# Mattdl/CLsurvey

Hardware: AMD Instinct MI355X
Metric: images/sec (train+importance pass), EWC small_VGG9 Tiny-ImageNet task batch (higher is better)
Workload: dtype f32 (bf16x6 split operands on the conv fwd/bwd-data matrix products, fp32 accumulate); 1 GPU; EWC small_VGG9_cl_128_128, Tiny-ImageNet shapes (3x64x64, 20 classes), batch 200: train step + Fisher step (BASELINE configs[1]); batch=200, parallelism=1 GPU

## Files before the change

### clsurvey_amd/_lib.py

```python
import ctypes as C
import os

_HERE = os.path.dirname(os.path.abspath(__file__))
LIB_PATH = os.path.join(_HERE, "libclhip.so")

_p = C.c_void_p
_i = C.c_int
_f = C.c_float
_z = C.c_size_t
_l = C.c_long


class HatParam(C.Structure):
    _fields_ = [("theta", _p), ("grad", _p), ("buf", _p), ("mask_back", _p), ("n", _z), ("is_emb", _i), ("reserved", _i)]


class HatGateJob(C.Structure):
    _fields_ = [("emb_row", _p), ("gate", _p), ("mask_pre", _p), ("n", _i), ("reserved", _i)]


class HatLayer(C.Structure):
    _fields_ = [("w", _p), ("gate_in", _p), ("out", _p), ("K", _z), ("C", _z), ("R", _z)]


# ... 99 lines not shown
    "clhip_hat_emb_grads_multi": (_i, [_p, _i, _f, _f, _f, _p, _p]),
    "clhip_pathnet_ws": (_z, [_p, _i]),
    "clhip_pathnet_pack_multi": (_i, [_p, _i, _p, _z, _p, _z, _p]),
    "clhip_pathnet_fold_grads_multi": (_i, [_p, _i, _p, _z, _p, _z, _p, _z, _p]),
    "clhip_pathnet_sgd_step": (_i, [_p, _i, _p, _p, _p, _z, _f, _f, _f, _f, _i, _p, _z, _p]),
    "clhip_softmax_ce_slice": (_i, [_p, _p, _i, _i, _i, _i, _i, _p, _p, _p, _p]),
    "clhip_net_loss_step_slice": (_i, [_p, _p, _p, _p, _p, _i, _i, _i, _i, _p, _p, _p, _p, _p]),
    "clhip_axpy": (_i, [_p, _p, _z, _f, _i, _p]),
    "clhip_gem_gram_ws": (_z, [_i]),
    "clhip_gem_gram": (_i, [_p, _z, C.POINTER(_i), _i, _z, _p, _p, _z, _p]),
    "clhip_gem_project": (_i, [_p, _z, C.POINTER(_i), C.POINTER(_f), _i, _p, _p, _z, _p]),
    "clhip_gem_qp": (_i, [_p, _i, C.c_double, C.c_double, _p, _p, _p]),
    "clhip_gem_project_dev": (_i, [_p, _z, C.POINTER(_i), _p, _p, _i, _p, _p, _z, _p]),
    "clhip_net_create": (_i, [C.POINTER(LayerDesc), _i, _i, _i, _i, _i, C.POINTER(_p)]),
    "clhip_net_set_dropout": (_i, [_p, _i, _p, _l]),
    "clhip_net_set_bn": (_i, [_p, _i, _p, _p, _f, _f]),
    "clhip_net_set_training": (_i, [_p, _i]),
    "clhip_net_probe": (_i, [_p, _i]),
    "clhip_net_probe_read": (_i, [_p, C.POINTER(_f), C.POINTER(_i)]),
    "clhip_net_layer_input": (_i, [_p, _i, _p, _p]),
    "clhip_net_layer_pool_idx": (_i, [_p, _i, _p, _p]),
    "clhip_net_prepared_weights": (_i, [_p, _p, _p]),
    "clhip_net_edge_grid_count": (_i, [_p]),
    "clhip_net_layer_paths": (_i, [_p, _i]),
    "clhip_net_probe_kind": (_i, [_p, _i, _i]),
    "clhip_net_set_input_grad": (_i, [_p, _i, _p]),
    "clhip_sigmoid_fwd": (_i, [_p, _p, _z, _p]),
    "clhip_sigmoid_bwd": (_i, [_p, _p, _p, _z, _p]),
    "clhip_mse_mean": (_i, [_p, _p, _z, _f, _p, _p, _p]),
    "clhip_adadelta_step": (_i, [_p, _p, _p, _p, _z, _f, _f, _f, _f, _p]),
    "clhip_bn_ws": (_z, [_i]),
    "clhip_bn_fwd": (_i, [_p, _p, _p, _p, _p, _p, _p, _p, _i, _i, _i, _i, _f, _f, _i, _p, _z, _p]),
    "clhip_bn_bwd": (_i, [_p, _p, _p, _p, _p, _p, _p, _p, _p, _i, _i, _i, _i, _i, _p, _z, _p]),
    "clhip_net_destroy": (None, [_p]),
    "clhip_net_workspace_bytes": (_z, [_p]),
    "clhip_net_num_classes": (_i, [_p]),
    "clhip_net_forward": (_i, [_p, _p, _p, _i, _p, _p, _p]),
    "clhip_net_backward": (_i, [_p, _p, _p, _p, _i, _p, _p, _p]),
    "clhip_net_loss_step": (_i, [_p, _p, _p, _p, _p, _i, _i, _p, _p, _p, _p, _p]),
    "clhip_rehearsal_assemble": (_i, [_p, _p, _i, _z, _p, _p, _l, _l, _i, _p, _i, _p, _p, _p]),
    "clhip_rehearsal_assemble_crop_flip": (_i, [_p, _p, _i, _i, _i, _i, _i, _i, _p, _l, _p, _p, _p, _l, _l, _i, _p, _p, _i, _p, _p, _p]),
    "clhip_rehearsal_assemble_resized_crop_flip": (_i, [_p, _p, _i, _i, _i, _i, _i, _i, _p, _l, _p, _p, _p, _l, _l, _i, _p, _p, _i, _p, _p, _p]),
    "clhip_loss_segments": (_i, [_p, _p, _p, _i, _i, _i, _p, _i, _f, _p, _p, _p, _p]),
    "clhip_net_loss_step_loss_segments": (_i, [_p, _p, _p, _p, _p, _p, _i, _i, _p, _i, _f, _p, _p, _p, _p, _p]),
    "clhip_gather_tasks": (_i, [_p, _i, _z, _p, _i, _p, _p, _p]),
    "clhip_slice_argmax_count": (_i, [_p, _i, _i, _p, _i, _p, _p, _p, _p, _p]),
# ... 52 lines not shown
```

### clsurvey_amd/csrc/common.hpp

```cpp
#pragma once
#include <hip/hip_runtime.h>
#include <stdint.h>
#include <stddef.h>
#include "../../include/clhip.h"

#define CLHIP_LAUNCH_CHECK()                          \
    do {                                              \
        hipError_t e__ = hipGetLastError();           \
        if (e__ != hipSuccess) return (int)e__;       \
    } while (0)

static inline hipStream_t as_stream(void* s) { return reinterpret_cast<hipStream_t>(s); }

static inline bool aligned16(const void* p) { return (reinterpret_cast<uintptr_t>(p) & 15u) == 0; }

static inline int ew_grid(size_t work_items, int block) {
    size_t g = (work_items + block - 1) / block;
    if (g < 1) g = 1;
    if (g > 2048) g = 2048;
    return (int)g;
}

static __device__ __attribute__((aligned(16))) float clhip_zero16[4] = {0.f, 0.f, 0.f, 0.f};

// ... 100 lines not shown
int clhip_internal_fc_fwd_partial(const float* x, const float* w, int M, int I, int O, void* ws, size_t ws_bytes, int* live,
                                  hipStream_t s);

#define CLHIP_WGRAD_JOBS_MAX 32
struct clhip_wgrad_job { const float* part; float* dw; float* db; int K, C, splits; int taps; };
int clhip_internal_conv3x3_wgrad_partial(const float* x, const float* dy, const uint8_t* unpool_idx, float* dw, float* db, int N,
                                         int C, int K, int H, int W, void* ws, size_t ws_bytes, void* stream, clhip_wgrad_job* job);
int clhip_internal_wgrad_reduce_multi(const clhip_wgrad_job* jobs, int n, hipStream_t s);

bool clhip_internal_convkk_ok(int N, int Cin, int Cout, int H, int W, int R, int S, int stride, int pad);
int clhip_internal_convkk(int mode, const float* in, const float* w, const float* bias, const float* mask_src, float* out, int N,
                          int Cin, int Cout, int H, int W, int relu, hipStream_t s);

struct clhip_wino_wt { const float* w; float* U; int Ko, Ci, mode, pad; };
int clhip_internal_wino_weights(const clhip_wino_wt* jobs, int n, hipStream_t s);
int clhip_internal_weight_images(const clhip_wino_wt* wino_jobs, int n_wino, const clhip_wino_wt* bs_jobs, int n_bs, hipStream_t s);
int clhip_internal_c3w64_pool_weight_images(const float* x, const float* w, const float* b, float* y_pool, uint8_t* idx_u8, int N, int C,
                                            int K, int H, int W, const clhip_wino_wt* wino_jobs, int n_wino, const clhip_wino_wt* bs_jobs,
                                            int n_bs, int wt_first, hipStream_t s);
int clhip_internal_wino_conv_u(int mode, const float* in, const float* U, const float* bias, const float* mask_src, float* out,
                               uint8_t* pool_idx, int unpool, int N, int Cin, int Cout, int H, int W, int relu, hipStream_t s);
bool clhip_internal_wino_ok(int Cin, int Cout, int H, int W);
size_t clhip_internal_wino_ws(int Cin, int Cout);
bool clhip_internal_bs_ok(int Cin, int Cout, int H, int W);
bool clhip_internal_bs_preferred(int Cin, int Cout, int H, int W);
bool clhip_internal_bs5_preferred(int Cin, int Cout, int H, int W);
size_t clhip_internal_bs5_ws(int Cin, int Cout);
int clhip_internal_bs5_conv_u(int mode, const float* in, const void* wimg, const float* bias, const float* mask_src, float* out, int N,
                              int Cin, int Cout, int H, int W, int relu, hipStream_t s);
size_t clhip_internal_bs_ws(int Cin, int Cout);
int clhip_internal_bs_weights(const clhip_wino_wt* jobs, int n, hipStream_t s);
int clhip_internal_bs_conv_u(int mode, const float* in, const void* wimg, const float* bias, const float* mask_src, float* out,
                             uint8_t* pool_idx, int unpool, int N, int Cin, int Cout, int H, int W, int relu, hipStream_t s);
bool clhip_internal_bs5_wgrad_ok(int N, int C, int K, int H, int W);
size_t clhip_internal_bs5_wgrad_ws(int N, int C, int K, int H, int W);
int clhip_internal_bs5_wgrad(const float* x, const float* dy, float* dw, float* db, int N, int C, int K, int H, int W, void* ws,
                             size_t ws_bytes, hipStream_t s);
size_t clhip_internal_bs3k_wgrad_ws(int N, int C, int K, int H, int W);
int clhip_internal_bs3k_wgrad(const float* x, const float* dy, float* dw, float* db, int N, int C, int K, int H, int W, void* ws,
                              size_t ws_bytes, hipStream_t s);
bool clhip_internal_bs_wgrad_ok(int C, int K, int H, int W);
bool clhip_internal_bs_wgrad_preferred(int C, int K, int H, int W, int pooled);
size_t clhip_internal_bs_wgrad_ws(int N, int C, int K, int H, int W);
int clhip_internal_bs_wgrad_partial(const float* x, const float* dy, const uint8_t* unpool_idx, float* dw, float* db, int N, int C, int K,
                                    int H, int W, void* ws, size_t ws_bytes, hipStream_t s, clhip_wgrad_job* job);
bool clhip_internal_wino_wgrad_ok(int C, int K, int H, int W);
// ... 11 lines not shown
```

### clsurvey_amd/csrc/engine.hip

```cpp
#include <vector>
#include <cstdlib>
#include <new>
#include "common.hpp"

namespace {

struct LayerPlan {
    int type;
    int cin, cout, relu, pool;
    long w_off, b_off;
    int h, w;
    int ks, st, pd;
    int oh, ow;
    int pk, ps;
    int ph, pw;
    size_t in_elems, out_elems, pool_elems;
    size_t act_off;
    size_t pool_off;
    size_t idx_off;
    int bn;
    long bn_w_off, bn_b_off;
    size_t z_off;
    size_t stat_off;
    float* rmean; float* rvar; float bn_momentum, bn_eps;
// ... 10 lines not shown
    const float* extra_grad;
    const float* drop;
    long drop_stride;
    int has_drop_buf;
    size_t drop_off;
};

constexpr long long WINO_MIN_UNITS = 640;
constexpr long long WINO16_MIN_UNITS = 384;
static bool wino_small_wgrad() { return true; }

static bool wino_enabled() {
    const char* e = std::getenv("CLHIP_WINO");
    return !(e && e[0] == '0');
}

constexpr unsigned PROBE_RING = 64;
#ifndef CLHIP_EDGE_GRIDS_DEFAULT
#define CLHIP_EDGE_GRIDS_DEFAULT 1
#endif
#ifndef CLHIP_OVERLAP_DEFAULT
#define CLHIP_OVERLAP_DEFAULT 0
#endif

struct NetPlan {
    std::vector<LayerPlan> layers;
    int max_batch, in_c, in_h, in_w, n_classes;
    size_t in_elems;
    size_t acts_floats;
    size_t idx_bytes;
    size_t grad_floats;
    size_t scratch_bytes;
    size_t wino_bytes;
    size_t off_wino;
    size_t off_s2d;
    int s2d_fresh_n;
    size_t total_bytes;
    size_t off_acts, off_idx, off_g0, off_g1, off_scratch, off_dlogits, off_loss, off_fcdz, off_wg;
    int training;
    int n_wg;
    int fc_first;
    bool fc_fused;
    clhip_fc_chain chain;
    int probe_layer;
    int probe_kind;
    unsigned probe_count;
    std::vector<hipEvent_t> probe_ev;
    bool fc_tail, no_combo;
    unsigned* tail_counter;
    size_t off_rows;
    int edge_grids;
    unsigned edge_count;
    bool overlap;
    int overlap_mode;
    hipStream_t side;
    std::vector<hipEvent_t> ev_dy, ev_wg;
    ~NetPlan() {
        for (hipEvent_t e : ev_dy) (void)hipEventDestroy(e);
        for (hipEvent_t e : ev_wg) (void)hipEventDestroy(e);
        if (side) (void)hipStreamDestroy(side);
        if (tail_counter) (void)hipFree(tail_counter);
        for (hipEvent_t e : probe_ev) (void)hipEventDestroy(e);
    }
};

inline size_t align_up(size_t v, size_t a) { return (v + a - 1) / a * a; }

__global__ void drop_scale_kernel(float* __restrict__ h, const float* __restrict__ mask, long stride, int feat, size_t total) {
    for (size_t i = blockIdx.x * (size_t)blockDim.x + threadIdx.x; i < total; i += (size_t)gridDim.x * blockDim.x) {
        const size_t n = i / feat, f = i - n * feat;
        h[i] *= mask[n * stride + f];
    }
}

__global__ void add_inplace_kernel(float* __restrict__ a, const float* __restrict__ b, size_t n) {
// ... 209 lines not shown
    p->total_bytes = off;
    p->training = 1;
    p->overlap = false;
    p->side = nullptr;
    const char* ov = getenv("CLHIP_WGRAD_OVERLAP");
    bool any_bn = false;
    for (const LayerPlan& L : p->layers) any_bn = any_bn || L.bn;
    p->overlap_mode = (ov && ov[0] == '1') ? 1 : (ov && ov[0] == '2') ? 2 : CLHIP_OVERLAP_DEFAULT;
    if (p->overlap_mode && !any_bn) {
        if (hipStreamCreateWithFlags(&p->side, hipStreamNonBlocking) == hipSuccess) {
            p->overlap = true;
            p->ev_dy.resize(n_layers); p->ev_wg.resize(n_layers);
            for (int i = 0; i < n_layers && p->overlap; ++i)
                if (hipEventCreateWithFlags(&p->ev_dy[i], hipEventDisableTiming) != hipSuccess ||
                    hipEventCreateWithFlags(&p->ev_wg[i], hipEventDisableTiming) != hipSuccess) p->overlap = false;
        } else {
            (void)hipGetLastError();
            p->side = nullptr;
        }
    }
    p->edge_count = 0;
    const char* eg = getenv("CLHIP_EDGE_GRIDS");
    p->edge_grids = (eg && eg[0] >= '0' && eg[0] <= '2' && !eg[1]) ? eg[0] - '0' : CLHIP_EDGE_GRIDS_DEFAULT;
    p->probe_layer = -1;
    p->probe_kind = 0;
    p->probe_count = 0;
    p->fc_tail = false;
    p->no_combo = false;
    p->tail_counter = nullptr;
    const char* tl = getenv("CLHIP_FC_TAIL");
    if (tl && tl[0] == '0') p->no_combo = true;
    if (p->fc_fused && !(tl && tl[0] == '0') && clhip_internal_fc_tail_ok(&p->chain) &&
        max_batch <= 1024) {
        if (hipMalloc(reinterpret_cast<void**>(&p->tail_counter), 256) == hipSuccess &&
            hipMemset(p->tail_counter, 0, 256) == hipSuccess) {
            p->fc_tail = true;
        } else {
            (void)hipGetLastError();
            if (p->tail_counter) { (void)hipFree(p->tail_counter); p->tail_counter = nullptr; }
        }
    }
    *out_handle = p;
    return 0;
}

int clhip_net_set_dropout(void* handle, int layer, const float* mask, long row_stride) {
// ... 16 lines not shown
    NetPlan* p = static_cast<NetPlan*>(handle);
    if (!p || layer <= 0 || layer >= (int)p->layers.size() || !ws_float_off || !in_elems) return CLHIP_EINVAL;
    const LayerPlan& P = p->layers[layer - 1];
    *ws_float_off = p->off_acts / sizeof(float) + ((P.type == 0 && P.pool) ? P.pool_off : P.act_off);
    *in_elems = p->layers[layer].in_elems;
    return 0;
}

int clhip_net_layer_pool_idx(void* handle, int layer, size_t* ws_byte_off, size_t* elems) {
    NetPlan* p = static_cast<NetPlan*>(handle);
    if (!p || layer < 0 || layer >= (int)p->layers.size() || !ws_byte_off || !elems) return CLHIP_EINVAL;
    const LayerPlan& L = p->layers[layer];
    if (L.type != 0 || !L.pool) return CLHIP_EINVAL;
    *ws_byte_off = p->off_idx + L.idx_off;
    *elems = L.pool_elems;
    return 0;
}

int clhip_net_edge_grid_count(void* handle) {
    NetPlan* p = static_cast<NetPlan*>(handle);
    return p ? (int)(p->edge_count & 0x7fffffffu) : CLHIP_EINVAL;
}

int clhip_net_prepared_weights(void* handle, size_t* ws_byte_off, size_t* bytes) {
    NetPlan* p = static_cast<NetPlan*>(handle);
    if (!p || !ws_byte_off || !bytes) return CLHIP_EINVAL;
    *ws_byte_off = p->off_wino;
    *bytes = p->wino_bytes;
    return 0;
}

int clhip_net_layer_paths(void* handle, int layer) {
    NetPlan* p = static_cast<NetPlan*>(handle);
    if (!p || layer < 0 || layer >= (int)p->layers.size()) return CLHIP_EINVAL;
    const LayerPlan& L = p->layers[layer];
    const bool defer_capable = p->n_wg > 0 && !(p->overlap && p->overlap_mode == 1);
    if (L.type == 1) {
        bool tail = p->fc_tail && layer > p->fc_first;
        for (size_t i = p->fc_first + 1; tail && i < p->layers.size(); ++i)
            if (p->layers[i].drop || p->layers[i].extra_grad) tail = false;
        return (tail ? 64 : 0) | ((p->fc_fused && layer >= p->fc_first) ? 128 : 0);
    }
    return (L.wino_f ? 1 : 0) | (L.wino_d ? 2 : 0) | ((L.wino_w && defer_capable) ? 4 : 0) | ((L.bs_f || L.bs5_f) ? 8 : 0) |
           ((L.bs_d || L.bs5_d) ? 16 : 0) | ((L.bs_w && defer_capable) ? 32 : 0);
}

// ... 81 lines not shown
}

static void wino_collect(const NetPlan* p, const float* params, char* base, bool fwd, bool bwd, std::vector<clhip_wino_wt>& jobs,
                         std::vector<clhip_wino_wt>& bsjobs) {
    jobs.reserve(2 * p->layers.size());
    bsjobs.reserve(2 * p->layers.size());
    for (const LayerPlan& L : p->layers) {
        if (L.type != 0) continue;
        if (fwd && L.wino_f)
            (L.bs_f ? bsjobs : jobs).push_back(clhip_wino_wt{params + L.w_off, reinterpret_cast<float*>(base + p->off_wino + L.wino_uf), L.cout, L.cin, 0, 0});
        if (bwd && L.wino_d)
            (L.bs_d ? bsjobs : jobs).push_back(clhip_wino_wt{params + L.w_off, reinterpret_cast<float*>(base + p->off_wino + L.wino_ud), L.cin, L.cout, 1, 0});
        if (fwd && L.bs5_f)
            bsjobs.push_back(clhip_wino_wt{params + L.w_off, reinterpret_cast<float*>(base + p->off_wino + L.wino_uf), L.cout, L.cin, 0, 5});
        if (bwd && L.bs5_d)
            bsjobs.push_back(clhip_wino_wt{params + L.w_off, reinterpret_cast<float*>(base + p->off_wino + L.wino_ud), L.cin, L.cout, 1, 5});
    }
}

static int wino_prepare(NetPlan* p, const float* params, char* base, bool fwd, bool bwd, hipStream_t s) {
    std::vector<clhip_wino_wt> jobs, bsjobs;
    wino_collect(p, params, base, fwd, bwd, jobs, bsjobs);
    return clhip_internal_weight_images(jobs.data(), (int)jobs.size(), bsjobs.data(), (int)bsjobs.size(), s);
}

static int net_forward_impl(void* handle, const float* params, const float* x, int N, void* ws, float* logits_out,
                            void* stream, int tail, int* slabs_live = nullptr, bool prep_bwd = false) {
    NetPlan* p = static_cast<NetPlan*>(handle);
    if (!p || !params || !x || !ws || N <= 0 || N > p->max_batch) return CLHIP_EINVAL;
    char* base = static_cast<char*>(ws);
    float* acts = reinterpret_cast<float*>(base + p->off_acts);
    uint8_t* idx = reinterpret_cast<uint8_t*>(base + p->off_idx);
    void* scratch = base + p->off_scratch;
    std::vector<clhip_wino_wt> edge_jobs, edge_bsjobs;
    bool edge = false;
    if (p->wino_bytes) {
        const LayerPlan& L0 = p->layers[0];
        edge = p->edge_grids && L0.type == 0 && L0.ks == 3 && L0.st == 1 && L0.pd == 1 && !L0.bn && L0.pool && L0.pk == 2 && L0.ps == 2 &&
               L0.relu && !L0.wino_f && !L0.drop && L0.cin == 3;
        if (edge) {
            wino_collect(p, params, base, true, prep_bwd, edge_jobs, edge_bsjobs);
        } else {
            int rcw = wino_prepare(p, params, base, true, prep_bwd, as_stream(stream));
            if (rcw) return rcw;
        }
    }
    const float* cur = x;
    int rc;
    const size_t n_run = tail ? (size_t)p->fc_first + 1 : p->layers.size();
    int live = 0;
    for (size_t li = 0; li < n_run; ++li) {
        const LayerPlan& L = p->layers[li];
        float* y = acts + L.act_off;
        const bool probed = (int)li == p->probe_layer && p->probe_kind == 0 && !p->probe_ev.empty();
        if (probed) (void)hipEventRecord(p->probe_ev[2 * (p->probe_count % PROBE_RING)], as_stream(stream));
        struct ProbeEnd {
            NetPlan* p; bool on; hipStream_t s;
            ~ProbeEnd() { if (on) { (void)hipEventRecord(p->probe_ev[2 * (p->probe_count % PROBE_RING) + 1], s); ++p->probe_count; } }
        } probe_end{p, probed, as_stream(stream)};
        if (L.drop && L.has_drop_buf) {
            float* dropped = acts + L.drop_off;
            rc = drop_copy(cur, dropped, L.drop, L.drop_stride, L.in_elems, N, as_stream(stream));
            if (rc) return rc;
            cur = dropped;
        } else if (L.drop) {
            rc = drop_scale(const_cast<float*>(cur), L.drop, L.drop_stride, L.in_elems, N, as_stream(stream));
            if (rc) return rc;
        }
        const bool vgg = L.type == 0 && L.ks == 3 && L.st == 1 && L.pd == 1;
        const bool pool22 = L.pool && L.pk == 2 && L.ps == 2;
        if (L.type == 0 && (L.bn || !(vgg && (!L.pool || pool22)))) {
            float* zc = L.bn ? acts + L.z_off : y;
            const int crelu = L.bn ? 0 : L.relu;
            rc = (vgg && L.wino_f)
// ... 456 lines not shown
```

### clsurvey_amd/csrc/wino.hip

```cpp
#include "common.hpp"
#include "weight_images.hpp"
#include <cstdlib>

namespace {


struct WGeoW {
    static constexpr int TCB = 4, TRB = 4, NIMG = 4;
    static constexpr int PW = 2 * TCB + 2;
    static constexpr int PR = 2 * TRB + 2;
    static constexpr int PLANE = NIMG * PR * PW;
    static constexpr int X_FLOATS = WCK * PLANE;
    static constexpr int BUF = W_FLOATS + X_FLOATS;
};

__global__ __launch_bounds__(256) void wino_weight_kernel(const float* __restrict__ w, float* __restrict__ U, int Ko, int Ci,
                                                          int mode, int n_chunks) {
    const int total = ((Ko + WKT - 1) / WKT) * n_chunks * WCK * WKT;
    for (int i = blockIdx.x * 256 + threadIdx.x; i < total; i += gridDim.x * 256) {
        const int k_l = i % WKT, c_l = (i / WKT) % WCK, chunk = (i / (WKT * WCK)) % n_chunks, kt = i / (WKT * WCK * n_chunks);
        const int k = kt * WKT + k_l, c = chunk * WCK + c_l;
        float g[3][3];
#pragma unroll
        for (int r = 0; r < 3; ++r)
// ... 553 lines not shown
            }
        }
    }
    if (ct == 0 && wc == 0) {
        bsum += __shfl_xor(bsum, 32, 64);
        const int k = k0 + wk * 32 + li;
        if (kk == 0 && k < K) clhip_buf_store(bsum, rs_slab, (int)(9 * K * C + k) * 4, 0);
    }
}


typedef float floatx4v __attribute__((ext_vector_type(4)));

template <bool UNPOOL, int KT2>
constexpr bool wino16_adirect = !(UNPOOL && KT2 == 2);

template <bool UNPOOL, int KT2>
__host__ __device__ constexpr int wino16_lds_floats() {
    return 2 * ((wino16_adirect<UNPOOL, KT2> ? 0 : W_FLOATS) + WCK * KT2 * 100) + WKT;
}

template <int MODE, bool UNPOOL, int KT2>
__device__ __forceinline__ void wino_conv16_body(
    float* __restrict__ lds, const int bid,
    const float* __restrict__ in, const float* __restrict__ U, const float* __restrict__ bias,
    const float* __restrict__ mask_src, float* __restrict__ out, uint8_t* __restrict__ pool_idx,
    int N, int Cin, int Cout, int relu) {
    constexpr int H = 8, W = 8, NIMG = KT2;
    constexpr int PW = 10, PR = 10, PLANE = NIMG * PR * PW;
    constexpr bool ADIRECT = wino16_adirect<UNPOOL, KT2>;
    constexpr int WOFF = ADIRECT ? 0 : W_FLOATS;
    constexpr int X_FLOATS = WCK * PLANE, BUF = WOFF + X_FLOATS;
    static_assert(wino16_lds_floats<UNPOOL, KT2>() == 2 * BUF + WKT, "LDS size of the wrappers");
    float* const bias_s = lds + 2 * BUF;
    const int tid = threadIdx.x, lane = tid & 63, wave = tid >> 6;
    const int wk = KT2 == 2 ? wave & 1 : wave, wp = KT2 == 2 ? wave >> 1 : 0;
    constexpr int KW = 16 * KT2;
    const int ti = lane & 15, q = lane >> 4;
    const int n_grp = (N + NIMG - 1) / NIMG;
    const int kt = bid / n_grp, ng = bid - kt * n_grp;
    const int n0 = ng * NIMG, ko0 = kt * WKT;
    const int n_chunks = (Cin + WCK - 1) / WCK;
    if (MODE == 0 && tid < WKT) bias_s[tid] = (bias && ko0 + tid < Cout) ? bias[ko0 + tid] : 0.f;

    constexpr int Hi = UNPOOL ? H >> 1 : H, Wi = UNPOOL ? W >> 1 : W;
    constexpr int plane_in = Hi * Wi;
    const float* in_blk = in + (size_t)n0 * Cin * plane_in;
    const __amdgpu_buffer_rsrc_t rs_x = clhip_rsrc(in_blk, (size_t)(N - n0) * Cin * plane_in * sizeof(float));
    const __amdgpu_buffer_rsrc_t rs_i = clhip_rsrc(UNPOOL ? pool_idx + (size_t)n0 * Cin * plane_in : pool_idx,
                                                   UNPOOL ? (size_t)(N - n0) * Cin * plane_in : 0);
    const __amdgpu_buffer_rsrc_t rs_u = ADIRECT
        ? clhip_rsrc(U + (size_t)((Cout + WKT - 1) / WKT) * n_chunks * W_FLOATS + (size_t)kt * 2 * n_chunks * WD_FLOATS,
                     (size_t)2 * n_chunks * WD_FLOATS * sizeof(float))
        : clhip_rsrc(U + (size_t)kt * n_chunks * W_FLOATS, (size_t)n_chunks * W_FLOATS * sizeof(float));

    constexpr int W_IT = ADIRECT ? 0 : W_FLOATS / 4 / 256;
    constexpr int X_IT = (X_FLOATS + 255) / 256;
    constexpr int NU = W_IT + X_IT;
// ... 184 lines not shown
                }
                continue;
            }
        }
        if (ok) {
            const size_t o = ((size_t)n * Cout + k) * chw + (size_t)oh * W + ow;
            if (MODE == 1 && mask_src) {
                const float2 m0 = *reinterpret_cast<const float2*>(mask_src + o), m1 = *reinterpret_cast<const float2*>(mask_src + o + W);
                y00 = m0.x > 0.f ? y00 : 0.f; y01 = m0.y > 0.f ? y01 : 0.f;
                y10 = m1.x > 0.f ? y10 : 0.f; y11 = m1.y > 0.f ? y11 : 0.f;
            }
            st2(o, y00, y01);
            st2(o + W, y10, y11);
        }
    }
}

template <int MODE, bool UNPOOL, int KT2>
__global__ __launch_bounds__(256, (wino16_adirect<UNPOOL, KT2> ? 2 : 1)) void wino_conv16_kernel(
    const float* __restrict__ in, const float* __restrict__ U, const float* __restrict__ bias,
    const float* __restrict__ mask_src, float* __restrict__ out, uint8_t* __restrict__ pool_idx,
    int N, int Cin, int Cout, int relu) {
    __shared__ __attribute__((aligned(16))) float lds[wino16_lds_floats<UNPOOL, KT2>()];
    wino_conv16_body<MODE, UNPOOL, KT2>(lds, (int)blockIdx.x, in, U, bias, mask_src, out, pool_idx, N, Cin, Cout, relu);
}


template <int TC, int TR, int EROWS>
__host__ __device__ constexpr int wino16g_lds_floats() {
    return 2 * 4 * (2 * TR / EROWS) * (2 * EROWS + 2) * (2 * TC + 2) + WKT;
}

template <int TC, int TR, int EROWS, int MODE, bool UNPOOL>
__device__ __forceinline__ void wino_conv16g_body(
    float* __restrict__ lds, const int bid,
    const float* __restrict__ in, const float* __restrict__ U, const float* __restrict__ bias,
    const float* __restrict__ mask_src, float* __restrict__ out, uint8_t* __restrict__ pool_idx,
    int N, int Cin, int Cout, int H, int W, int relu, int tiles_w, int tiles_h, int n_pix_blocks) {
    static_assert(TC * TR == 16, "16 tiles per wave");
    constexpr int CQ = 4;
    constexpr int NE = 2 * TR / EROWS;
    static_assert(NE * EROWS == 2 * TR && (NE == 1 || !UNPOOL || EROWS == 4), "whole entities");
    constexpr int PW = 2 * TC + 2, PRE = 2 * EROWS + 2, PLANE = NE * PRE * PW;
    constexpr int X_FLOATS = CQ * PLANE, BUF = X_FLOATS;
    static_assert(wino16g_lds_floats<TC, TR, EROWS>() == 2 * BUF + WKT, "LDS size of the wrappers");
    float* const bias_s = lds + 2 * BUF;
    const int tid = threadIdx.x, lane = tid & 63, wave = tid >> 6;
    const int wk = wave & 1, wp = wave >> 1;
    const int ti = lane & 15, q = lane >> 4;
    const int kt = bid / n_pix_blocks, pb = bid - kt * n_pix_blocks;
    const int bw = pb % tiles_w, v0 = (pb / tiles_w) * NE;
    const int nb0 = v0 / tiles_h, w0 = bw * 2 * TC;
    const int ko0 = kt * WKT;
    const int n_chunks = Cin / CQ;
    if (MODE == 0 && tid < WKT) bias_s[tid] = (bias && ko0 + tid < Cout) ? bias[ko0 + tid] : 0.f;

    const int Hi = UNPOOL ? H >> 1 : H, Wi = UNPOOL ? W >> 1 : W;
    const int plane_in = Hi * Wi;
    const float* in_img = in + (size_t)nb0 * Cin * plane_in;
    const __amdgpu_buffer_rsrc_t rs_x = clhip_rsrc(in_img, (size_t)(N - nb0) * Cin * plane_in * sizeof(float));
    const __amdgpu_buffer_rsrc_t rs_i = clhip_rsrc(UNPOOL ? pool_idx + (size_t)nb0 * Cin * plane_in : pool_idx,
                                                   UNPOOL ? (size_t)(N - nb0) * Cin * plane_in : 0);
    const __amdgpu_buffer_rsrc_t rs_u =
        clhip_rsrc(U + (size_t)((Cout + WKT - 1) / WKT) * (Cin / WCK) * W_FLOATS + (size_t)kt * n_chunks * WD_FLOATS,
                   (size_t)n_chunks * WD_FLOATS * sizeof(float));

    constexpr int X_IT = (X_FLOATS + 255) / 256;
    struct Stage {
        float4 wv[1];
        float xr[X_IT];
// ... 192 lines not shown
            st1(o, y00);
            if (col1) st1(o + 1, y01);
            if (row1) st1(o + W, y10);
            if (row1 && col1) st1(o + W + 1, y11);
        } else if (ok) {
            const size_t o = ((size_t)n * Cout + k) * chw + (size_t)oh * W + ow;
            if (MODE == 1 && mask_src) {
                const float2 m0 = *reinterpret_cast<const float2*>(mask_src + o), m1 = *reinterpret_cast<const float2*>(mask_src + o + W);
                y00 = m0.x > 0.f ? y00 : 0.f; y01 = m0.y > 0.f ? y01 : 0.f;
                y10 = m1.x > 0.f ? y10 : 0.f; y11 = m1.y > 0.f ? y11 : 0.f;
            }
            st2(o, y00, y01);
            st2(o + W, y10, y11);
        }
    }
}

template <int TC, int TR, int EROWS, int MODE, bool UNPOOL>
__global__ __launch_bounds__(256, 2) void wino_conv16g_kernel(
    const float* __restrict__ in, const float* __restrict__ U, const float* __restrict__ bias,
    const float* __restrict__ mask_src, float* __restrict__ out, uint8_t* __restrict__ pool_idx,
    int N, int Cin, int Cout, int H, int W, int relu, int tiles_w, int tiles_h, int n_pix_blocks) {
    __shared__ __attribute__((aligned(16))) float lds[wino16g_lds_floats<TC, TR, EROWS>()];
    wino_conv16g_body<TC, TR, EROWS, MODE, UNPOOL>(lds, (int)blockIdx.x, in, U, bias, mask_src, out, pool_idx, N, Cin, Cout, H, W, relu,
                                                   tiles_w, tiles_h, n_pix_blocks);
}


#ifndef CLHIP_WINO16_BELOW_UNITS
#define CLHIP_WINO16_BELOW_UNITS 640
#endif
constexpr long long WINO16_BELOW_UNITS = CLHIP_WINO16_BELOW_UNITS;


template <int TCS, int TRS>
struct WGeoP {
    static_assert(TCS * TRS == 16 && (TCS & (TCS - 1)) == 0, "16 tiles per stage, tile of a step by shifts");
    static constexpr int KB = 32, CB = 32;
    static constexpr int DW = 2 * TCS, DR = 2 * TRS;
    static constexpr int DPIX = DR * DW;
    static constexpr int PW = DW + 2, PR = DR + 2;
    static constexpr int PLANE = PR * PW;
    static constexpr int LDP = DPIX + 2;
    static constexpr int PLANEP = (PLANE % 4 == 2) ? PLANE : PLANE + 2;
    static_assert((LDP / 2) % 2 == 1 && (PLANEP / 2) % 2 == 1, "lane strides must be odd in 8-byte units");
    static constexpr int DY_FLOATS = KB * LDP, X_FLOATS = CB * PLANEP;
    static constexpr int BUF = DY_FLOATS + X_FLOATS;
// ... 284 lines not shown
}

template <int TCS, int TRS, bool UNPOOL, bool VEC>
__global__ __launch_bounds__(256, 2) void wino_wgrad_ps_kernel(
    const float* __restrict__ x, const float* __restrict__ dy, float* __restrict__ part, const uint8_t* __restrict__ unpool_idx,
    int N, int C, int K, int H, int W, int tiles_w, int tiles_h, int total_stages, int splits, int c_tiles, size_t slab_stride) {
    __shared__ __attribute__((aligned(16))) float lds[WGeoP<TCS, TRS>::LDS_FLOATS];
    wino_wgrad_ps_body<TCS, TRS, UNPOOL, VEC>(lds, (int)blockIdx.x, x, dy, part, unpool_idx, N, C, K, H, W, tiles_w, tiles_h,
                                              total_stages, splits, c_tiles, slab_stride);
}

template <int DK, int TC, int TR, int EROWS, bool UNPOOL, int TCS, int TRS>
__global__ __launch_bounds__(256, 2) void wino_pair_kernel(
    const float* __restrict__ d_in, const float* __restrict__ d_U, const float* __restrict__ d_mask, float* __restrict__ d_out,
    uint8_t* __restrict__ d_idx, int N, int d_Cin, int d_Cout, int H, int W, int d_tiles_w, int d_tiles_h, int d_npb,
    const float* __restrict__ w_x, float* __restrict__ w_part, int w_tiles_w, int w_tiles_h, int w_total, int w_splits, int w_ctiles,
    size_t w_slab, int nb_w) {
    constexpr int LD = DK ? wino16_lds_floats<UNPOOL, 1>() : wino16g_lds_floats<TC, TR, EROWS>(), LW = WGeoP<TCS, TRS>::LDS_FLOATS;
    __shared__ __attribute__((aligned(16))) float lds[LD > LW ? LD : LW];
    const int b = (int)blockIdx.x;
    const int kind = b < nb_w ? 1 : 0, idx = kind ? b : b - nb_w;
    if (kind == 0) {
        if constexpr (DK)
            wino_conv16_body<1, UNPOOL, 1>(lds, idx, d_in, d_U, nullptr, d_mask, d_out, d_idx, N, d_Cin, d_Cout, 0);
        else
            wino_conv16g_body<TC, TR, EROWS, 1, UNPOOL>(lds, idx, d_in, d_U, nullptr, d_mask, d_out, d_idx, N, d_Cin, d_Cout, H, W, 0,
                                                        d_tiles_w, d_tiles_h, d_npb);
    } else
        wino_wgrad_ps_body<TCS, TRS, UNPOOL, true>(lds, idx, w_x, d_in, w_part, d_idx, N, d_Cout, d_Cin, H, W, w_tiles_w, w_tiles_h,
                                                   w_total, w_splits, w_ctiles, w_slab);
}

template <int MODE, bool UNPOOL>
int launch_wino(const float* in, const float* U, const float* bias, const float* mask_src, float* out, uint8_t* pool_idx,
                int N, int Cin, int Cout, int H, int W, int relu, hipStream_t s) {
    const int kts = (Cout + WKT - 1) / WKT;
    if (H == 8 && W == 8 && ((long long)N * 16 + 31) / 32 * ((Cout + 31) / 32) < WINO16_BELOW_UNITS) {
        const bool narrow = (long long)N * ((Cout + 31) / 32) <= 512;
        const long long blocks = (long long)(narrow ? N : (N + 1) / 2) * kts;
        if (blocks <= 0 || blocks > 0x7fffffffLL) return CLHIP_EINVAL;
        if (narrow)
            hipLaunchKernelGGL((wino_conv16_kernel<MODE, UNPOOL, 1>), dim3((unsigned)blocks), dim3(256), 0, s, in, U, bias, mask_src, out,
                               pool_idx, N, Cin, Cout, relu);
        else
            hipLaunchKernelGGL((wino_conv16_kernel<MODE, UNPOOL, 2>), dim3((unsigned)blocks), dim3(256), 0, s, in, U, bias, mask_src, out,
                               pool_idx, N, Cin, Cout, relu);
        CLHIP_LAUNCH_CHECK();
        return 0;
    }
#define WINO_16G(TC_, TR_, ER_, UNP_)                                                                                          \
    do {                                                                                                                       \
        const int tiles_w = ((W + 1) / 2 + TC_ - 1) / TC_, groups = ((H + 1) / 2 + ER_ - 1) / ER_;                              \
        constexpr int NE_ = 2 * TR_ / ER_;                                                                                      \
// ... 210 lines not shown
    hipLaunchKernelGGL((wino_pair_kernel<DK_, TC_, TR_, 4, UNP_, TC_, TR_>), dim3((unsigned)(nb_d + nb_w)), dim3(256), 0, s, dy, U,  \
                       mask_src, dx, idx, N, K, C, H, W, d_tiles_w, d_groups, (int)npb, x, part, g.tiles_w, g.tiles_h, (int)g.total, \
                       (int)g.splits, C / 32, g.slab, (int)nb_w)
    if (wide) { if (unpool_idx) PAIR(0, 8, 2, true); else PAIR(0, 8, 2, false); }
    else if (narrow) { if (unpool_idx) PAIR(1, 4, 4, true); else PAIR(1, 4, 4, false); }
    else { if (unpool_idx) PAIR(0, 4, 4, true); else PAIR(0, 4, 4, false); }
#undef PAIR
    CLHIP_LAUNCH_CHECK();
    *job = clhip_wgrad_job{part, dw, db, K, C, (int)g.splits};
    return 0;
}

bool clhip_internal_wino_pair_shape(int N, int C, int K, int H, int W, int pooled) {
    if (N <= 0 || ((H | W) & 1) || (long long)H * W > CLHIP_PAIR_MAX_PIXELS || !clhip_internal_wino_ok(K, C, H, W)) return false;
    const bool wide = W >= 16, m88 = H == 8 && W == 8;
    if (!wide && !m88) return false;
    WgradGeo g;
    alignas(16) static const float a16[4] = {0.f, 0.f, 0.f, 0.f};
    static const uint8_t one = 0;
    if (wino_wgrad_geo(a16, a16, pooled ? &one : nullptr, N, C, K, H, W, (size_t)1 << 40, &g)) return false;
    return g.ps && g.vec && g.wide == wide;
}

extern "C" {

size_t clhip_conv3x3_wino_ws(int C, int K) {
    const size_t a = clhip_internal_wino_ws(C, K), b = clhip_internal_wino_ws(K, C);
    return a > b ? a : b;
}

int clhip_conv3x3_wino_fwd(const float* x, const float* w, const float* b, float* y, uint8_t* idx_u8_or_null, int N, int C, int K,
                           int H, int W, int relu, void* ws, size_t ws_bytes, void* stream) {
    if (N <= 0 || !clhip_internal_wino_ok(C, K, H, W)) return CLHIP_ENOTSUP;
    return clhip_internal_wino_conv(0, x, w, b, nullptr, y, idx_u8_or_null, 0, N, C, K, H, W, relu, ws, ws_bytes, as_stream(stream));
}

int clhip_conv3x3_wino_bwd_data(const float* dy, const uint8_t* idx_u8_or_null, const float* w, const float* relu_src, float* dx,
                                int N, int C, int K, int H, int W, void* ws, size_t ws_bytes, void* stream) {
    if (N <= 0 || !clhip_internal_wino_ok(K, C, H, W)) return CLHIP_ENOTSUP;
    return clhip_internal_wino_conv(1, dy, w, nullptr, relu_src, dx, const_cast<uint8_t*>(idx_u8_or_null), idx_u8_or_null != nullptr,
                                    N, K, C, H, W, 0, ws, ws_bytes, as_stream(stream));
}


size_t clhip_conv3x3_wino_bwd_weight_ws(int N, int C, int K, int H, int W) {
    const size_t a = clhip_internal_wino_wgrad_ws(N, C, K, H, W), b = clhip_conv3x3_bwd_weight_ws(N, C, K, H, W);
// ... 42 lines not shown
```

### clsurvey_amd/net.py

```python
import ctypes as C
import weakref

import torch
import torch.nn as nn

from . import _lib
from ._lib import check, LayerDesc


def _pad4(n):
    return (n + 3) // 4 * 4


class ParamArena:
    _registry = weakref.WeakValueDictionary()

    @classmethod
    def find(cls, params):
        params = list(params)
        if not params:
            return None
        a = cls._registry.get(id(params[0]))
        if a is None or len(a.params) != len(params) or any(x is not y for x, y in zip(a.params, params)):
            return None
# ... 211 lines not shown

    def layer_input(self, layer, n):
        off, elems = C.c_size_t(), C.c_size_t()
        check(_lib.lib().clhip_net_layer_input(self._h, int(layer), C.byref(off), C.byref(elems)), "clhip_net_layer_input")
        lo = off.value * 4
        return self.ws[lo:lo + n * elems.value * 4].view(torch.float32).view(n, elems.value)

    def pool_idx(self, layer, n):
        off, elems = C.c_size_t(), C.c_size_t()
        check(_lib.lib().clhip_net_layer_pool_idx(self._h, int(layer), C.byref(off), C.byref(elems)), "clhip_net_layer_pool_idx")
        return self.ws[off.value:off.value + n * elems.value].view(n, elems.value)

    def prepared_weights(self):
        off, nbytes = C.c_size_t(), C.c_size_t()
        check(_lib.lib().clhip_net_prepared_weights(self._h, C.byref(off), C.byref(nbytes)), "clhip_net_prepared_weights")
        return self.ws[off.value:off.value + nbytes.value]

    def edge_grid_count(self):
        n = _lib.lib().clhip_net_edge_grid_count(self._h)
        if n < 0:
            raise RuntimeError("clhip_net_edge_grid_count")
        return n

    def layer_paths(self, layer):
        bits = _lib.lib().clhip_net_layer_paths(self._h, int(layer))
        if bits < 0:
            raise RuntimeError("clhip_net_layer_paths(%d)" % layer)
        return {"fwd": bool(bits & 1), "bwd_data": bool(bits & 2), "bwd_weight": bool(bits & 4),
                "bs_fwd": bool(bits & 8), "bs_bwd_data": bool(bits & 16), "bs_bwd_weight": bool(bits & 32),
                "fc_tail": bool(bits & 64), "fc_fused": bool(bits & 128)}

    def set_input_grad(self, layer, extra):
        if extra is not None and (not extra.is_cuda or extra.dtype != torch.float32 or not extra.is_contiguous()):
            raise RuntimeError("set_input_grad needs a contiguous fp32 HIP tensor")
        self._extra = extra
        check(_lib.lib().clhip_net_set_input_grad(self._h, int(layer), extra.data_ptr() if extra is not None else None),
              "clhip_net_set_input_grad")

    def _mode(self):
        if not self.bns:
            return
        training = bool(self.model.training)
        if training != self._training:
            check(_lib.lib().clhip_net_set_training(self._h, int(training)), "clhip_net_set_training")
            self._training = training
        if training:
# ... 84 lines not shown
```

### include/clhip.h

```cpp
#ifndef CLHIP_H
#define CLHIP_H

#include <stddef.h>
#include <stdint.h>

#ifdef __cplusplus
extern "C" {
#endif

#if defined(__GNUC__) || defined(__clang__)
#pragma GCC visibility push(default)
#define CLHIP_VISIBILITY_PUSHED 1
#endif

#define CLHIP_EINVAL (-1)
#define CLHIP_ENOSPC (-2)
#define CLHIP_ENOTSUP (-3)

int clhip_sigmoid_fwd(const float* x, float* y, size_t n, void* stream);
int clhip_sigmoid_bwd(const float* dy, const float* y, float* dx, size_t n, void* stream);
int clhip_mse_mean(const float* a, const float* b, size_t n, float grad_scale, float* da, float* loss_out, void* stream);
int clhip_adadelta_step(float* theta, const float* grad, float* square_avg, float* acc_delta, size_t n, float lr, float rho,
                        float eps, float weight_decay, void* stream);

// ... 182 lines not shown
typedef struct {
    int type;
    int cin, cout;
    int relu, pool;
    long w_off, b_off;
    int ksize, stride, pad;
    int pool_k, pool_s;
    int bn;
    long bn_w_off, bn_b_off;
    int has_drop;
} clhip_layer_desc;

int clhip_net_create(const clhip_layer_desc* layers, int n_layers, int max_batch, int in_c, int in_h,
                     int in_w, void** out_handle);
int clhip_net_set_dropout(void* handle, int layer, const float* mask, long row_stride);
int clhip_net_set_bn(void* handle, int layer, float* running_mean, float* running_var, float momentum, float eps);
int clhip_net_set_training(void* handle, int training);
int clhip_net_probe(void* handle, int layer);
int clhip_net_probe_kind(void* handle, int layer, int kind);
int clhip_net_probe_read(void* handle, float* avg_us, int* count);
int clhip_net_layer_pool_idx(void* handle, int layer, size_t* ws_byte_off, size_t* elems_per_sample);
int clhip_net_prepared_weights(void* handle, size_t* ws_byte_off, size_t* bytes);
int clhip_net_edge_grid_count(void* handle);
int clhip_net_layer_paths(void* handle, int layer);

int clhip_net_layer_input(void* handle, int layer, size_t* ws_float_off, size_t* in_elems);
int clhip_net_set_input_grad(void* handle, int layer, const float* extra);
void clhip_net_destroy(void* handle);
size_t clhip_net_workspace_bytes(void* handle);
int clhip_net_num_classes(void* handle);
int clhip_net_forward(void* handle, const float* params, const float* x, int N, void* ws,
                      float* logits_out, void* stream);
int clhip_net_backward(void* handle, const float* params, float* grads, const float* x, int N, void* ws,
                       const float* dlogits, void* stream);
int clhip_net_loss_step(void* handle, const float* params, float* grads, const float* x,
                        const int64_t* labels_i64, int N, int loss_kind, void* ws, float* loss_out,
                        double* stats, float* logits_out, void* stream);

int clhip_net_loss_step_slice(void* handle, const float* params, float* grads, const float* x,
                              const int64_t* labels_i64, int N, int loss_kind, int col_off, int ncols, void* ws,
                              float* loss_out, double* stats, float* logits_out, void* stream);

int clhip_axpy(float* y, const float* x, size_t n, float alpha, int assign, void* stream);
size_t clhip_gem_gram_ws(int m);
int clhip_gem_gram(const float* G, size_t ld, const int* row_idx_host, int m, size_t n, double* out_f64, void* ws,
                   size_t ws_bytes, void* stream);
// ... 105 lines not shown
```

Measured before the change: 302,500 images/s.

## Fuse consecutive small Winograd forward conv layers into one per-image chain kernel

```diff
diff --git a/clsurvey_amd/_lib.py b/clsurvey_amd/_lib.py
--- a/clsurvey_amd/_lib.py
+++ b/clsurvey_amd/_lib.py
@@ -145,6 +145,7 @@
     "clhip_net_layer_pool_idx": (_i, [_p, _i, _p, _p]),
     "clhip_net_prepared_weights": (_i, [_p, _p, _p]),
     "clhip_net_edge_grid_count": (_i, [_p]),
+    "clhip_net_fwd_chain_count": (_i, [_p]),
     "clhip_net_layer_paths": (_i, [_p, _i]),
     "clhip_net_probe_kind": (_i, [_p, _i, _i]),
     "clhip_net_set_input_grad": (_i, [_p, _i, _p]),
diff --git a/clsurvey_amd/csrc/common.hpp b/clsurvey_amd/csrc/common.hpp
--- a/clsurvey_amd/csrc/common.hpp
+++ b/clsurvey_amd/csrc/common.hpp
@@ -146,6 +146,10 @@
                                uint8_t* pool_idx, int unpool, int N, int Cin, int Cout, int H, int W, int relu, hipStream_t s);
 bool clhip_internal_wino_ok(int Cin, int Cout, int H, int W);
 size_t clhip_internal_wino_ws(int Cin, int Cout);
+#define CLHIP_WINO_CHAIN_MAX 4
+struct clhip_wino_chain_layer { const float* in; const float* U; const float* bias; float* out; uint8_t* pool_idx; int Cin, Cout, H, W, relu; };
+int clhip_internal_wino_chain_kind(int N, int Cin, int Cout, int H, int W);
+int clhip_internal_wino_chain(const clhip_wino_chain_layer* layers, int n, int N, hipStream_t s);
 bool clhip_internal_bs_ok(int Cin, int Cout, int H, int W);
 bool clhip_internal_bs_preferred(int Cin, int Cout, int H, int W);
 bool clhip_internal_bs5_preferred(int Cin, int Cout, int H, int W);
diff --git a/clsurvey_amd/csrc/engine.hip b/clsurvey_amd/csrc/engine.hip
--- a/clsurvey_amd/csrc/engine.hip
+++ b/clsurvey_amd/csrc/engine.hip
@@ -56,6 +56,9 @@
 #ifndef CLHIP_OVERLAP_DEFAULT
 #define CLHIP_OVERLAP_DEFAULT 0
 #endif
+#ifndef CLHIP_FWD_CHAIN_DEFAULT
+#define CLHIP_FWD_CHAIN_DEFAULT 1
+#endif
 
 struct NetPlan {
     std::vector<LayerPlan> layers;
@@ -85,6 +88,8 @@
     size_t off_rows;
     int edge_grids;
     unsigned edge_count;
+    int fwd_chain;
+    int chain_count;
     bool overlap;
     int overlap_mode;
     hipStream_t side;
@@ -340,6 +345,9 @@
     p->edge_count = 0;
     const char* eg = getenv("CLHIP_EDGE_GRIDS");
     p->edge_grids = (eg && eg[0] >= '0' && eg[0] <= '2' && !eg[1]) ? eg[0] - '0' : CLHIP_EDGE_GRIDS_DEFAULT;
+    p->chain_count = 0;
+    const char* fc = getenv("CLHIP_FWD_CHAIN");
+    p->fwd_chain = (fc && (fc[0] == '0' || fc[0] == '1') && !fc[1]) ? fc[0] - '0' : CLHIP_FWD_CHAIN_DEFAULT;
     p->probe_layer = -1;
     p->probe_kind = 0;
     p->probe_count = 0;
@@ -402,6 +410,11 @@
     return p ? (int)(p->edge_count & 0x7fffffffu) : CLHIP_EINVAL;
 }
 
+int clhip_net_fwd_chain_count(void* handle) {
+    NetPlan* p = static_cast<NetPlan*>(handle);
+    return p ? p->chain_count : CLHIP_EINVAL;
+}
+
 int clhip_net_prepared_weights(void* handle, size_t* ws_byte_off, size_t* bytes) {
     NetPlan* p = static_cast<NetPlan*>(handle);
     if (!p || !ws_byte_off || !bytes) return CLHIP_EINVAL;
@@ -529,6 +542,22 @@
     std::vector<clhip_wino_wt> jobs, bsjobs;
     wino_collect(p, params, base, fwd, bwd, jobs, bsjobs);
     return clhip_internal_weight_images(jobs.data(), (int)jobs.size(), bsjobs.data(), (int)bsjobs.size(), s);
+}
+
+static int fwd_chain_run(const NetPlan* p, size_t li, size_t n_run, int N) {
+    if (!p->fwd_chain) return 0;
+    int n = 0;
+    for (size_t i = li; i < n_run && n < CLHIP_WINO_CHAIN_MAX; ++i) {
+        const LayerPlan& L = p->layers[i];
+        if (L.type != 0 || L.ks != 3 || L.st != 1 || L.pd != 1 || L.bn || !L.wino_f || L.bs_f) break;
+        if (L.drop || L.has_drop_buf || L.extra_grad) break;
+        if (L.pool && !(L.pk == 2 && L.ps == 2 && L.relu)) break;
+        if (clhip_internal_wino_chain_kind(N, L.cin, L.cout, L.h, L.w) < 0) break;
+        ++n;
+    }
+    if (n < 2) return 0;
+    if (p->probe_kind == 0 && !p->probe_ev.empty() && p->probe_layer >= (int)li && p->probe_layer < (int)li + n) return -n;
+    return n;
 }
 
 static int net_forward_impl(void* handle, const float* params, const float* x, int N, void* ws, float* logits_out,
@@ -556,7 +585,26 @@
     int rc;
     const size_t n_run = tail ? (size_t)p->fc_first + 1 : p->layers.size();
     int live = 0;
+    p->chain_count = 0;
+    size_t chain_from = 1;
     for (size_t li = 0; li < n_run; ++li) {
+        const int nc = li >= chain_from ? fwd_chain_run(p, li, n_run, N) : 0;
+        if (nc < 0) chain_from = li + (size_t)(-nc);
+        if (nc > 0) {
+            clhip_wino_chain_layer cl[CLHIP_WINO_CHAIN_MAX];
+            for (int j = 0; j < nc; ++j) {
+                const LayerPlan& Lj = p->layers[li + j];
+                float* oj = acts + (Lj.pool ? Lj.pool_off : Lj.act_off);
+                cl[j] = clhip_wino_chain_layer{cur, reinterpret_cast<const float*>(base + p->off_wino + Lj.wino_uf), params + Lj.b_off, oj,
+                                               Lj.pool ? idx + Lj.idx_off : nullptr, Lj.cin, Lj.cout, Lj.h, Lj.w, Lj.pool ? 1 : Lj.relu};
+                cur = oj;
+            }
+            rc = clhip_internal_wino_chain(cl, nc, N, as_stream(stream));
+            if (rc) return rc;
+            ++p->chain_count;
+            li += nc - 1;
+            continue;
+        }
         const LayerPlan& L = p->layers[li];
         float* y = acts + L.act_off;
         const bool probed = (int)li == p->probe_layer && p->probe_kind == 0 && !p->probe_ev.empty();
diff --git a/clsurvey_amd/csrc/wino.hip b/clsurvey_amd/csrc/wino.hip
--- a/clsurvey_amd/csrc/wino.hip
+++ b/clsurvey_amd/csrc/wino.hip
@@ -599,7 +599,7 @@
 
 template <int MODE, bool UNPOOL, int KT2>
 __device__ __forceinline__ void wino_conv16_body(
-    float* __restrict__ lds, const int bid,
+    float* __restrict__ lds, const int bid, const int vtid,
     const float* __restrict__ in, const float* __restrict__ U, const float* __restrict__ bias,
     const float* __restrict__ mask_src, float* __restrict__ out, uint8_t* __restrict__ pool_idx,
     int N, int Cin, int Cout, int relu) {
@@ -610,7 +610,7 @@
     constexpr int X_FLOATS = WCK * PLANE, BUF = WOFF + X_FLOATS;
     static_assert(wino16_lds_floats<UNPOOL, KT2>() == 2 * BUF + WKT, "LDS size of the wrappers");
     float* const bias_s = lds + 2 * BUF;
-    const int tid = threadIdx.x, lane = tid & 63, wave = tid >> 6;
+    const int tid = vtid, lane = tid & 63, wave = tid >> 6;
     const int wk = KT2 == 2 ? wave & 1 : wave, wp = KT2 == 2 ? wave >> 1 : 0;
     constexpr int KW = 16 * KT2;
     const int ti = lane & 15, q = lane >> 4;
@@ -841,7 +841,7 @@
     const float* __restrict__ mask_src, float* __restrict__ out, uint8_t* __restrict__ pool_idx,
     int N, int Cin, int Cout, int relu) {
     __shared__ __attribute__((aligned(16))) float lds[wino16_lds_floats<UNPOOL, KT2>()];
-    wino_conv16_body<MODE, UNPOOL, KT2>(lds, (int)blockIdx.x, in, U, bias, mask_src, out, pool_idx, N, Cin, Cout, relu);
+    wino_conv16_body<MODE, UNPOOL, KT2>(lds, (int)blockIdx.x, (int)threadIdx.x, in, U, bias, mask_src, out, pool_idx, N, Cin, Cout, relu);
 }
 
 
@@ -852,7 +852,7 @@
 
 template <int TC, int TR, int EROWS, int MODE, bool UNPOOL>
 __device__ __forceinline__ void wino_conv16g_body(
-    float* __restrict__ lds, const int bid,
+    float* __restrict__ lds, const int bid, const int vtid,
     const float* __restrict__ in, const float* __restrict__ U, const float* __restrict__ bias,
     const float* __restrict__ mask_src, float* __restrict__ out, uint8_t* __restrict__ pool_idx,
     int N, int Cin, int Cout, int H, int W, int relu, int tiles_w, int tiles_h, int n_pix_blocks) {
@@ -864,7 +864,7 @@
     constexpr int X_FLOATS = CQ * PLANE, BUF = X_FLOATS;
     static_assert(wino16g_lds_floats<TC, TR, EROWS>() == 2 * BUF + WKT, "LDS size of the wrappers");
     float* const bias_s = lds + 2 * BUF;
-    const int tid = threadIdx.x, lane = tid & 63, wave = tid >> 6;
+    const int tid = vtid, lane = tid & 63, wave = tid >> 6;
     const int wk = wave & 1, wp = wave >> 1;
     const int ti = lane & 15, q = lane >> 4;
     const int kt = bid / n_pix_blocks, pb = bid - kt * n_pix_blocks;
@@ -1103,7 +1103,7 @@
     const float* __restrict__ mask_src, float* __restrict__ out, uint8_t* __restrict__ pool_idx,
     int N, int Cin, int Cout, int H, int W, int relu, int tiles_w, int tiles_h, int n_pix_blocks) {
     __shared__ __attribute__((aligned(16))) float lds[wino16g_lds_floats<TC, TR, EROWS>()];
-    wino_conv16g_body<TC, TR, EROWS, MODE, UNPOOL>(lds, (int)blockIdx.x, in, U, bias, mask_src, out, pool_idx, N, Cin, Cout, H, W, relu,
+    wino_conv16g_body<TC, TR, EROWS, MODE, UNPOOL>(lds, (int)blockIdx.x, (int)threadIdx.x, in, U, bias, mask_src, out, pool_idx, N, Cin, Cout, H, W, relu,
                                                    tiles_w, tiles_h, n_pix_blocks);
 }
 
@@ -1434,13 +1434,49 @@
     const int kind = b < nb_w ? 1 : 0, idx = kind ? b : b - nb_w;
     if (kind == 0) {
         if constexpr (DK)
-            wino_conv16_body<1, UNPOOL, 1>(lds, idx, d_in, d_U, nullptr, d_mask, d_out, d_idx, N, d_Cin, d_Cout, 0);
+            wino_conv16_body<1, UNPOOL, 1>(lds, idx, (int)threadIdx.x, d_in, d_U, nullptr, d_mask, d_out, d_idx, N, d_Cin, d_Cout, 0);
         else
-            wino_conv16g_body<TC, TR, EROWS, 1, UNPOOL>(lds, idx, d_in, d_U, nullptr, d_mask, d_out, d_idx, N, d_Cin, d_Cout, H, W, 0,
+            wino_conv16g_body<TC, TR, EROWS, 1, UNPOOL>(lds, idx, (int)threadIdx.x, d_in, d_U, nullptr, d_mask, d_out, d_idx, N, d_Cin, d_Cout, H, W, 0,
                                                         d_tiles_w, d_tiles_h, d_npb);
     } else
         wino_wgrad_ps_body<TCS, TRS, UNPOOL, true>(lds, idx, w_x, d_in, w_part, d_idx, N, d_Cout, d_Cin, H, W, w_tiles_w, w_tiles_h,
                                                    w_total, w_splits, w_ctiles, w_slab);
+}
+
+constexpr int WINO_CHAIN_MAX = CLHIP_WINO_CHAIN_MAX;
+struct WinoChainLayer {
+    const float* in; const float* U; const float* bias; float* out; uint8_t* pool_idx;
+    int Cin, Cout, relu, kind;
+};
+struct WinoChain { int n, N; WinoChainLayer l[WINO_CHAIN_MAX]; };
+
+__global__ __launch_bounds__(512, 1) void wino_chain_kernel(const WinoChain C) {
+    constexpr int L0 = wino16g_lds_floats<8, 2, 4>(), L1 = wino16_lds_floats<false, 1>(), LV = ((L0 > L1 ? L0 : L1) + 3) & ~3;
+    __shared__ __attribute__((aligned(16))) float lds[2 * LV];
+    const int vb = __builtin_amdgcn_readfirstlane((int)threadIdx.x >> 8), vtid = (int)threadIdx.x & 255;
+    const int img = (int)blockIdx.x, N = C.N;
+    float* const my = lds + vb * LV;
+    auto handoff = [](int i, int& t) {
+        if (i) {
+            __builtin_amdgcn_fence(__ATOMIC_RELEASE, "workgroup");
+            __syncthreads();
+        }
+        asm volatile("" : "+v"(t));
+    };
+    int i = 0;
+    for (; i < C.n && C.l[i].kind == 0; ++i) {
+        const WinoChainLayer& q = C.l[i];
+        int t = vtid;
+        handoff(i, t);
+        wino_conv16g_body<8, 2, 4, 0, false>(my, 2 * img + vb, t, q.in, q.U, q.bias, nullptr, q.out, q.pool_idx, N, q.Cin, q.Cout,
+                                             16, 16, q.relu, 1, 2, 2 * N);
+    }
+    for (; i < C.n; ++i) {
+        const WinoChainLayer& q = C.l[i];
+        int t = vtid;
+        handoff(i, t);
+        wino_conv16_body<0, false, 1>(my, vb * N + img, t, q.in, q.U, q.bias, nullptr, q.out, q.pool_idx, N, q.Cin, q.Cout, q.relu);
+    }
 }
 
 template <int MODE, bool UNPOOL>
@@ -1697,6 +1733,32 @@
     return g.ps && g.vec && g.wide == wide;
 }
 
+int clhip_internal_wino_chain_kind(int N, int Cin, int Cout, int H, int W) {
+    if (N <= 0 || !clhip_internal_wino_ok(Cin, Cout, H, W)) return -1;
+    if (H == 16 && W == 16 && Cout == WKT) return 0;
+    if (H == 8 && W == 8 && Cout == 2 * WKT && ((long long)N * 16 + 31) / 32 * ((Cout + 31) / 32) < WINO16_BELOW_UNITS &&
+        (long long)N * 2 <= 0x7fffffffLL)
+        return 1;
+    return -1;
+}
+
+int clhip_internal_wino_chain(const clhip_wino_chain_layer* layers, int n, int N, hipStream_t s) {
+    if (!layers || n < 1 || n > WINO_CHAIN_MAX || N <= 0) return CLHIP_EINVAL;
+    WinoChain C;
+    C.n = n; C.N = N;
+    for (int i = 0; i < n; ++i) {
+        const clhip_wino_chain_layer& q = layers[i];
+        const int kind = clhip_internal_wino_chain_kind(N, q.Cin, q.Cout, q.H, q.W);
+        if (!q.in || !q.U || !q.out || kind < 0) return CLHIP_EINVAL;
+        if (i && kind < C.l[i - 1].kind) return CLHIP_EINVAL;
+        C.l[i] = WinoChainLayer{q.in, q.U, q.bias, q.out, q.pool_idx, q.Cin, q.Cout, q.relu, kind};
+    }
+    for (int i = n; i < WINO_CHAIN_MAX; ++i) C.l[i] = WinoChainLayer{nullptr, nullptr, nullptr, nullptr, nullptr, 0, 0, 0, 0};
+    hipLaunchKernelGGL(wino_chain_kernel, dim3((unsigned)N), dim3(512), 0, s, C);
+    CLHIP_LAUNCH_CHECK();
+    return 0;
+}
+
 extern "C" {
 
 size_t clhip_conv3x3_wino_ws(int C, int K) {
diff --git a/clsurvey_amd/net.py b/clsurvey_amd/net.py
--- a/clsurvey_amd/net.py
+++ b/clsurvey_amd/net.py
@@ -257,6 +257,12 @@
             raise RuntimeError("clhip_net_edge_grid_count")
         return n
 
+    def fwd_chain_count(self):
+        n = _lib.lib().clhip_net_fwd_chain_count(self._h)
+        if n < 0:
+            raise RuntimeError("clhip_net_fwd_chain_count")
+        return n
+
     def layer_paths(self, layer):
         bits = _lib.lib().clhip_net_layer_paths(self._h, int(layer))
         if bits < 0:
diff --git a/include/clhip.h b/include/clhip.h
--- a/include/clhip.h
+++ b/include/clhip.h
@@ -228,6 +228,7 @@
 int clhip_net_layer_pool_idx(void* handle, int layer, size_t* ws_byte_off, size_t* elems_per_sample);
 int clhip_net_prepared_weights(void* handle, size_t* ws_byte_off, size_t* bytes);
 int clhip_net_edge_grid_count(void* handle);
+int clhip_net_fwd_chain_count(void* handle);
 int clhip_net_layer_paths(void* handle, int layer);
 
 int clhip_net_layer_input(void* handle, int layer, size_t* ws_float_off, size_t* in_elems);
```

Result: no change. 304,300 images/s (median of 6 runs) (+0.6%).
